# OpenStitching/stitching

Hardware: AMD Instinct MI355X
Metric: warped+blended Mpix/s (higher is better)
Workload: dtype u8/int16 (fixed-point remap, int32 pyramid sums, fp32 weights); 1 GPU; BASELINE config 2: 8 synthetic 4000x3000 frames, one ring; yaw step 38.9 deg = 0.58 hfov (42 % overlap; SURVEY 8(d) names 0.70 hfov); spherical warp + 5-band multiband blend, inputs resident in HBM; frames_per_gpu=8, panoramas_in_flight=2

## Files before the change

### include/stitching_amd_debug.h

```cpp
#ifndef STITCHING_AMD_DEBUG_H
#define STITCHING_AMD_DEBUG_H

#include "stitching_amd.h"

#ifdef __cplusplus
extern "C" {
#endif

int stx_debug_warp_maps(stx_ctx* ctx, int type, float scale, const float K[9], const float R[9], int w, int h, int which,
                        const int rect_xywh[4], stx_buf** out_xmap_f32, stx_buf** out_ymap_f32, int out_xywh[4]);

int stx_debug_feather_dist_cap(void);

#ifdef __cplusplus
}
#endif
#endif
```

### stitching_amd/_lib.py

```python
import ctypes as C
import os

from .stitching_error import StitchingError

_HERE = os.path.dirname(os.path.abspath(__file__))
LIB_PATH = os.environ.get("STITCHING_AMD_LIB") or os.path.join(_HERE, "libstitching_amd.so")

STX_OK = 0
WARP_PLANE, WARP_AFFINE, WARP_CYLINDRICAL, WARP_SPHERICAL = 0, 1, 2, 3
WARP_TYPE_IDS = {"plane": 0, "affine": 1, "cylindrical": 2, "spherical": 3, "fisheye": 4, "stereographic": 5,
                 "compressedPlaneA2B1": 6, "compressedPlaneA1.5B1": 7, "compressedPlanePortraitA2B1": 8,
                 "compressedPlanePortraitA1.5B1": 9, "paniniA2B1": 10, "paniniA1.5B1": 11, "paniniPortraitA2B1": 12,
                 "paniniPortraitA1.5B1": 13, "mercator": 14, "transverseMercator": 15}
INTER_NEAREST, INTER_LINEAR = 0, 1
BORDER_CONSTANT, BORDER_REFLECT = 0, 2
BLEND_NO, BLEND_FEATHER, BLEND_MULTIBAND = 0, 1, 2
U8, S16, F32 = 0, 1, 2
TRIG_MODES = {"exact": 0, "glibc": 1, "glibc-nofma": 2}
REMAP_MODES = {"q15": 0, "float": 1, "float-fma": 2}
PYRDOWN_MODES = {"scalar": 0, "simd-v": 1, "simd-hv": 3, "simd-v-fma": 5, "simd-hv-fma": 7}
GAIN_MAP_BOUNDED = 1
EXPOSURE_KINDS = {"gain": 1, "gain_blocks": 2, "channel": 3, "channel_blocks": 4}
EXPOSURE_SOLVERS = {"host": 0, "device": 1}
LU_NB, LU_MAX_N = 32, 16384
# ... 1 lines not shown
COLOR_SEAM_MAX_LENGTH, COLOR_SEAM_MAX_CROSS = 16384, 4096
FEATURES_MAX_SIDE, FEATURES_MAX_LEVELS, FEATURES_MAX_FEATURES = 32767, 16, 65536
MATCH_MAX_FEATURES, MATCH_MAX_ITERS = 65536, 4096
RAY_MAX_CAMERAS, RAY_MAX_MATCHES = 1024, 131072
CONTRIB_U8_BINARY = 1
STRIP_MASK_BITS = 2

EXPORTS = (
    "stx_version stx_last_error stx_set_trig_mode stx_get_trig_mode stx_set_remap_mode stx_get_remap_mode stx_set_pyrdown_mode stx_get_pyrdown_mode stx_device_count stx_ctx_create stx_ctx_destroy stx_ctx_sync "
    "stx_host_alloc stx_host_free stx_buf_from_host stx_buf_from_host_async stx_buf_alloc stx_buf_to_host stx_buf_to_host_async stx_buf_view stx_buf_info stx_buf_device_ptr stx_buf_free "
    "stx_warp_roi stx_warp_rois stx_warp stx_warp_image_and_mask stx_warp_batch stx_warp_batch_rects stx_warp_batch_gain stx_warp_batch_with_rois stx_warp_mask "
    "stx_gain_apply stx_block_gain_apply stx_block_gain_apply_batch stx_resize_linear_exact stx_resize_linear_exact_batch stx_seam_mask_resize stx_seam_mask_resize_batch stx_seam_mask_resize_batch_sub stx_timelapse_frame stx_result_roi stx_blend_create stx_blend_num_bands stx_blend_feed stx_blend_finish stx_blend_finish_ex "
    "stx_blend_destroy stx_blend_keep_weights stx_blend_use_weights stx_mb_weights_free stx_blend_set_band stx_blend_feed_ex stx_blend_contrib_rect stx_blend_export_contrib stx_blend_export_contribs "
    "stx_blend_build stx_blend_feed_contrib stx_blend_feed_contrib_ex stx_buf_flags stx_strip_rect stx_view_rect stx_strip_pack stx_strip_pack_batch stx_strip_pack_batch_ex stx_strip_bytes stx_strip_unpack stx_blend_feed_strips stx_comm_unique_id stx_comm_create stx_comm_exchange stx_comm_exchange_begin stx_comm_exchange_end stx_comm_exchange_begin_on stx_comm_exchange_end_on stx_comm_info stx_comm_destroy stx_prof_enable stx_prof_reset stx_prof_count stx_prof_get stx_mark stx_mark_elapsed_ms "
    "stx_exposure_feed stx_exposure_stats stx_exposure_solve stx_set_exposure_solver stx_get_exposure_solver stx_exposure_feed_ex stx_exposure_solve_device stx_lu_solve_device stx_seam_find stx_seam_schedule stx_color_seam_find stx_crop_lir stx_features_detect stx_match_features stx_ray_problem_create stx_ray_problem_eval stx_ray_problem_free "
    "stx_debug_warp_maps stx_debug_feather_dist_cap"
).split()

_lib = None


def build_hint():
    return "build it with `make -C stitching_amd/csrc` or `python -c 'import __graft_entry__ as g; g.build()'`"


def lib():
    global _lib
    if _lib is not None:
        return _lib
    if not os.path.exists(LIB_PATH):
        raise ImportError(f"{LIB_PATH} is missing: the HIP back end is not built ({build_hint()}). "
# ... 73 lines not shown
    L.stx_blend_feed_strips.argtypes = [vp, C.c_int, vpp, ip, ip, ip, ip, ip, C.c_int]
    L.stx_comm_unique_id.argtypes = [C.POINTER(C.c_ubyte)]
    L.stx_comm_create.argtypes = [vp, C.c_int, C.c_int, C.POINTER(C.c_ubyte), vpp]
    L.stx_comm_exchange.argtypes = [vp, C.c_int, ip, ip, C.POINTER(C.c_void_p), C.POINTER(C.c_size_t)]
    L.stx_comm_exchange_begin.argtypes = [vp, C.c_int, ip, ip, C.POINTER(C.c_void_p), C.POINTER(C.c_size_t)]
    L.stx_comm_exchange_end.argtypes = [vp]
    L.stx_comm_exchange_begin_on.argtypes = [vp, vp, C.c_int, ip, ip, C.POINTER(C.c_void_p), C.POINTER(C.c_size_t)]
    L.stx_comm_exchange_end_on.argtypes = [vp, vp]
    L.stx_comm_info.argtypes = [vp, ip]
    L.stx_comm_destroy.argtypes = [vp]
    L.stx_prof_enable.argtypes = [vp, C.c_int]
    L.stx_prof_reset.argtypes = [vp]
    L.stx_prof_count.argtypes = [vp, ip]
    L.stx_prof_get.argtypes = [vp, C.c_int, C.c_char_p, C.c_int, C.POINTER(C.c_int64), C.POINTER(C.c_double),
                               C.POINTER(C.c_double)]
    L.stx_debug_warp_maps.argtypes = [vp, C.c_int, C.c_float, fp, fp, C.c_int, C.c_int, C.c_int, ip, vpp, vpp, ip]
    llp, dp = C.POINTER(C.c_longlong), C.POINTER(C.c_double)
    L.stx_exposure_feed.argtypes = [vp, C.c_int, C.c_int, vpp, vpp, ip, C.c_int, C.c_int, dp, llp, dp]
    L.stx_exposure_stats.argtypes = [vp, C.c_int, C.c_int, vpp, vpp, ip, C.c_int, llp, ip, llp, dp]
    L.stx_exposure_solve.argtypes = [C.c_int, C.c_int, ip, dp, C.POINTER(C.c_ubyte), dp]
    L.stx_set_exposure_solver.argtypes = [C.c_int]
    L.stx_exposure_feed_ex.argtypes = [vp, C.c_int, C.c_int, vpp, vpp, ip, C.c_int, C.c_int, C.c_int, dp, llp, dp]
    L.stx_exposure_solve_device.argtypes = [vp, C.c_int, C.c_int, ip, dp, C.POINTER(C.c_ubyte), dp, dp]
    L.stx_lu_solve_device.argtypes = [vp, C.c_int, dp, dp, dp, dp]
    L.stx_seam_find.argtypes = [vp, C.c_int, C.c_int, ip, ip, vpp, vpp, dp]
    L.stx_seam_schedule.argtypes = [C.c_int, ip, ip, ip, ip, ip]
    L.stx_color_seam_find.argtypes = [vp, C.c_int, ip, ip, vpp, vpp, vpp, dp]
    L.stx_crop_lir.argtypes = [vp, vp, ip, ip, dp]
    L.stx_features_detect.argtypes = [vp, C.c_int, vpp, vpp, C.c_int, C.c_int, C.c_int, ip, ip, ip, ip, C.POINTER(C.c_byte), ip, ip, llp,
                                      C.POINTER(C.c_ubyte), dp]
# ... 19 lines not shown
```

### stitching_amd/csrc/stx_blend_fast.hip

```cpp
#include <algorithm>
#include <cstdlib>

#include "stx_blend_kernels.h"
#include "stx_device_math.h"

using namespace stxd;

namespace {

constexpr int L0_WAVES = 5;
constexpr float WEIGHT_EPS = 1e-5f;
constexpr float INV255 = 0.0039215688593685627f;
constexpr float INV256 = 0.00390625f;

#define STX_GAS __attribute__((address_space(1)))
template <class T> STX_DEV const STX_GAS T* gp(const T* p) { return (const STX_GAS T*)p; }
template <class T> STX_DEV STX_GAS T* gp(T* p) { return (STX_GAS T*)p; }

STX_DEV bool xcd_tile(const StxTileMap& M, uint32_t b, int& tx, int& ty)
{
    if (M.plain) {
        const uint32_t wy = M.tiles_x == 1 ? b : __umulhi(b, M.magic_tx);
        tx = (int)(b - wy * (uint32_t)M.tiles_x);
        ty = (int)wy;
// ... 929 lines not shown
        const uint32_t w0 = __builtin_amdgcn_alignbyte(d.y, d.x, sh), w1 = d.y >> (8u * sh);
        return ((w0 & (n >= 4 ? 0xffffffffu : (1u << (8 * n)) - 1u)) | (n > 4 ? w1 & 0xffu : 0u)) != 0u;
    }
    const uint32_t d0 = q[0], d1 = q[1], d2 = q[2];
    const uint32_t w0 = __builtin_amdgcn_alignbyte(d1, d0, sh), w1 = __builtin_amdgcn_alignbyte(d2, d1, sh), w2 = d2 >> (8u * sh);
    const uint32_t m0 = n >= 4 ? 0xffffffffu : (1u << (8 * n)) - 1u;
    const uint32_t m1 = n >= 8 ? 0xffffffffu : (n > 4 ? (1u << (8 * (n - 4))) - 1u : 0u);
    return ((w0 & m0) | (w1 & m1) | (n > 8 ? w2 & 0xffu : 0u)) != 0u;
}
template <bool L0>
STX_DEV bool occ_hit(const StxMbImage& im, int lv, int tile_x, int Y0)
{
    return occ_hit_f<L0>(im.occ[L0 ? 1 : lv], im.fx, im.fy, im.fw, im.fh, lv, tile_x, Y0);
}

template <bool WF>
STX_DEV void level0_epilogue_pk(const MbLevelK& P, int X0, int Y0, uint32_t (&acc)[2][3][4], uint32_t (&cnt)[2][4], const float (*ws)[8]);

template <bool L0, bool CONTRIB, bool EMIT, bool U8SRC>
STX_DEV void mb_level_fast_body(const MbLevelK& P)
{
    const int tid = threadIdx.x;
    const int lv = P.level;
    int tile_tx, tile_ty;
    if (!xcd_tile(P.tiles, blockIdx.x, tile_tx, tile_ty)) return;
    const int tile_x = P.x0 + tile_tx * 512, tile_y = P.y0 + tile_ty * LV_TH;
    const int X0 = tile_x + (tid & 63) * 8, Y0 = tile_y + __builtin_amdgcn_readfirstlane(tid >> 6) * 2;
    const bool active = X0 < P.x1 && Y0 < P.y1;

    int acc[2][8][3];
// ... 502 lines not shown
                for (int c = 0; c < 3; c++) w[j][c] = half_of(j) ? s16hi(v[r][c][pair_of(j)]) : s16lo(v[r][c][pair_of(j)]);
            uint32_t t[12];
#pragma unroll
            for (int j = 0; j < 8; j += 2) {
                t[(j >> 1) * 3 + 0] = pack16(w[j][0], w[j][1]);
                t[(j >> 1) * 3 + 1] = pack16(w[j][2], w[j + 1][0]);
                t[(j >> 1) * 3 + 2] = pack16(w[j + 1][1], w[j + 1][2]);
            }
            *reinterpret_cast<uint4*>(p16) = make_uint4(t[0], t[1], t[2], t[3]);
            *reinterpret_cast<uint4*>(p16 + 4) = make_uint4(t[4], t[5], t[6], t[7]);
            *reinterpret_cast<uint4*>(p16 + 8) = make_uint4(t[8], t[9], t[10], t[11]);
        }
    }
}

template <bool CONTRIB, bool DEFER = false>
__global__ __launch_bounds__(LV_THREADS) __attribute__((amdgpu_waves_per_eu(L0_WAVES, 8))) void mb_level0_pk_kernel(MbLevelK P)
{
    const int tid = threadIdx.x;
    int tile_tx, tile_ty;
    if (!xcd_tile(P.tiles, blockIdx.x, tile_tx, tile_ty)) return;
    const int tile_x = P.x0 + tile_tx * 512, tile_y = P.y0 + tile_ty * LV_TH;
    const int X0 = tile_x + (tid & 63) * 8, Y0 = tile_y + __builtin_amdgcn_readfirstlane(tid >> 6) * 2;
    const bool active = X0 < P.x1 && Y0 < P.y1;

    uint32_t acc[2][3][4];
    uint32_t cntb[2][2];
#pragma unroll
    for (int r = 0; r < 2; r++) {
#pragma unroll
        for (int k = 0; k < 4; k++) acc[r][0][k] = acc[r][1][k] = acc[r][2][k] = 0;
        cntb[r][0] = cntb[r][1] = 0;
    }
    uint32_t grey_seen = 0u;

    for (int base = 0; base < P.n_images; base += 64) {
        bool hit = false;
        {
            const int kk = base + (tid & 63);
            const StxMbImage& im = P.images[min(kk, P.n_images - 1)];
            const v4u f = *reinterpret_cast<const v4u_a4*>(&im.iw);
            const v4u ff = *reinterpret_cast<const v4u_a4*>(&im.fx);
            const uint8_t* const occp = im.occ[1];
            const int kind = CONTRIB ? im.kind : 0;
            int rx = (int)f.z, ry = (int)f.w, rw = (int)f.x, rh = (int)f.y;
            if (CONTRIB && kind == 1) { rx = (int)ff.x; ry = (int)ff.y; rw = (int)ff.z; rh = (int)ff.w; }
            hit = (kk < P.n_images) & (rx < tile_x + 512) & (rx + rw > tile_x) & (ry < Y0 + 2) & (ry + rh > Y0);
            if (hit) hit = occ_hit_f<true>(occp, (int)ff.x, (int)ff.y, (int)ff.z, (int)ff.w, 0, tile_x, Y0);
        }
        unsigned long long todo = __ballot(hit);
        while (todo) {
            const int k = base + (int)__builtin_ctzll(todo);
            todo &= todo - 1;
            const StxMbImage& im = P.images[k];
            if (!active) continue;
            if (CONTRIB && im.kind == 1) {
                const int cx0 = X0 - im.fx, cy0 = Y0 - im.fy;
                if ((unsigned)cx0 >= (unsigned)im.fw || (unsigned)cy0 >= (unsigned)im.fh) continue;
#pragma unroll
                for (int r = 0; r < 2; r++) {
#pragma unroll
                    for (int c = 0; c < 3; c++) {
                        const v4u gv = *reinterpret_cast<const STX_GAS v4u*>(
                            gp(im.g[0]) + c * im.g_plane[0] + ((uint32_t)(cy0 + r) * (uint32_t)im.g_stride[0] + (uint32_t)cx0));
                        acc[r][c][0] = unpk(pk(acc[r][c][0]) + pk(__builtin_amdgcn_perm(gv.y, gv.x, 0x05040100u)));
// ... 178 lines not shown
                            acc[r][j][c] += trunc_small(fmul((float)L, w));
                        }
                        ws[r][j] = fadd(ws[r][j], w);
                    }
            }
            if (live) level_epilogue<true>(P, X0, Y0, acc, ws);
        }
        g0 += nb;
    }
}

STX_DEV uint32_t min3u(uint32_t a, uint32_t b, uint32_t c) { return min(min(a, b), c); }
STX_DEV uint32_t max3u(uint32_t a, uint32_t b, uint32_t c) { return max(max(a, b), c); }

constexpr int LVPK_WAVES = 3;
__global__ __launch_bounds__(LV_THREADS) __attribute__((amdgpu_waves_per_eu(LVPK_WAVES, 8))) void mb_level_pk_kernel(MbLevelK P)
{
    const int tid = threadIdx.x;
    const int lv = P.level;
    int tile_tx, tile_ty;
    if (!xcd_tile(P.tiles, blockIdx.x, tile_tx, tile_ty)) return;
    const int tile_x = P.x0 + tile_tx * 512, tile_y = P.y0 + tile_ty * LV_TH;
    const int X0 = tile_x + (tid & 63) * 8, Y0 = tile_y + __builtin_amdgcn_readfirstlane(tid >> 6) * 2;
    const bool active = X0 < P.x1 && Y0 < P.y1;

    uint32_t acc[2][3][4];
    float ws[2][8];
#pragma unroll
    for (int r = 0; r < 2; r++) {
#pragma unroll
        for (int q = 0; q < 4; q++) acc[r][0][q] = acc[r][1][q] = acc[r][2][q] = 0;
#pragma unroll
        for (int j = 0; j < 8; j++) ws[r][j] = 0.f;
    }
    uint32_t ones = 0;
    uint32_t mixed = 0;

    for (int base = 0; base < P.n_images; base += 64) {
        bool hit = false;
        {
            const int kk = base + (tid & 63);
            const StxMbImage& im = P.images[min(kk, P.n_images - 1)];
            const v4u f = *reinterpret_cast<const v4u_a4*>(&im.fx);
            const uint8_t* const occp = im.occ[lv];
            const int rx = (int)f.x >> lv, ry = (int)f.y >> lv, rw = (int)f.z >> lv, rh = (int)f.w >> lv;
            hit = (kk < P.n_images) & (rx < tile_x + 512) & (rx + rw > tile_x) & (ry < Y0 + 2) & (ry + rh > Y0);
            if (hit) hit = occ_hit_f<false>(occp, (int)f.x, (int)f.y, (int)f.z, (int)f.w, lv, tile_x, Y0);
        }
        unsigned long long todo = __ballot(hit);
        while (todo) {
            const int k = base + (int)__builtin_ctzll(todo);
            todo &= todo - 1;
            const StxMbImage& im = P.images[k];
            if (!active) continue;
            int i_fx = im.fx, i_fy = im.fy, i_fw = im.fw, i_fh = im.fh, i_w1h = im.w1_f16;
            unsigned long long W_a = (unsigned long long)im.wt[lv], G0_a = (unsigned long long)im.g[lv], G1_a = (unsigned long long)im.g[lv + 1];
            uint32_t wst = (uint32_t)im.wt_stride[lv], g0s = (uint32_t)im.g_stride[lv], g1s = (uint32_t)im.g_stride[lv + 1];
            uint32_t g0p = (uint32_t)im.g_plane[lv], g1p = (uint32_t)im.g_plane[lv + 1];
            asm("" : "+s"(i_fx), "+s"(i_fy), "+s"(i_fw), "+s"(i_fh), "+s"(i_w1h), "+s"(W_a), "+s"(G0_a), "+s"(G1_a), "+s"(wst), "+s"(g0s),
                "+s"(g1s), "+s"(g0p), "+s"(g1p));
            const int lx0 = X0 - (i_fx >> lv), ly0 = Y0 - (i_fy >> lv);
            const int lw = i_fw >> lv, lh = i_fh >> lv;
            if ((unsigned)lx0 >= (unsigned)lw || (unsigned)ly0 >= (unsigned)lh) continue;
            const bool w_half = lv == 1 && i_w1h != 0;
// ... 164 lines not shown
#pragma unroll
    for (int r = 0; r < 2; r++) {
        if (Y0 + r >= P.y1) break;
#pragma unroll
        for (int c = 0; c < 3; c++) {
            v4u o;
            o.x = __builtin_amdgcn_perm(v[r][c][2], v[r][c][0], 0x05040100u);
            o.y = __builtin_amdgcn_perm(v[r][c][2], v[r][c][0], 0x07060302u);
            o.z = __builtin_amdgcn_perm(v[r][c][3], v[r][c][1], 0x05040100u);
            o.w = __builtin_amdgcn_perm(v[r][c][3], v[r][c][1], 0x07060302u);
            *reinterpret_cast<STX_GAS v4u*>(gp(P.out) + c * P.out_plane + (long long)(Y0 + r - P.out_y0) * P.out_stride + (X0 - P.out_x0)) = o;
        }
    }
}

bool launched_ok() { return hipGetLastError() == hipSuccess; }

}

bool stx_fast_mb_down_batch(stx_ctx* ctx, const StxMbImage* d_images, const StxMbImage* h_images, int n, int level, bool weights)
{
    int mw = 0, mh = 0;
    for (int i = 0; i < n; i++) {
        mw = std::max(mw, (h_images[i].fw >> level) >> 1);
        mh = std::max(mh, (h_images[i].fh >> level) >> 1);
    }
    if (n <= 0 || mw < 1 || mh < 1 || n > 65535) return false;
    StxTileMap M = stx_tile_map((mw + DN_TOW - 1) / DN_TOW, (mh + DN_TOH - 1) / DN_TOH, DN_BAND);
    constexpr int DN_PLAIN_FROM = 3;
    M.plain = level >= DN_PLAIN_FROM;
// ... 39 lines not shown
    return launched_ok();
}

static bool no_defer()
{
    static const bool off = getenv("STITCHING_AMD_NO_DEFER") != nullptr;
    return off;
}

bool stx_fast_mb_level(stx_ctx* ctx, const MbLevelK& K)
{
    MbLevelK KT;
    if (!fast_level_ok(K, &KT)) return false;
    dim3 grid(stx_tile_grid(KT.tiles), 1);
    hipStream_t st = ctx->stream;
    if (K.level == 0 && K.pk_ok && !K.emit && K.num_bands > 0) {
        static const unsigned pad_lds = getenv("STITCHING_AMD_L0_LDS") ? (unsigned)atoi(getenv("STITCHING_AMD_L0_LDS")) : 0u;
        if (K.has_contrib) hipLaunchKernelGGL(mb_level0_pk_kernel<true>, grid, dim3(LV_THREADS), pad_lds, st, KT);
        else hipLaunchKernelGGL(mb_level0_pk_kernel<false>, grid, dim3(LV_THREADS), pad_lds, st, KT);
    } else if (K.level == 0 && K.all_u8 && !K.has_contrib && !K.emit && K.num_bands > 0 && !no_defer()) {
        const int segs = std::min(KT.tiles.tiles_x, STX_DEFER_SEGS);
        const size_t seg_cap = (size_t)((KT.tiles.tiles_x + STX_DEFER_SEGS - 1) / STX_DEFER_SEGS) * (size_t)KT.tiles.tiles_y * (unsigned)LV_THREADS;
        const size_t counters = (size_t)STX_DEFER_SEGS * 128;
        KT.defer_segs = segs;
        StxDevBlock q;
        if (stx_dev_alloc(ctx, counters + seg_cap * (size_t)segs * sizeof(unsigned long long), &q) != STX_OK) return false;
        KT.defer_count = reinterpret_cast<unsigned*>(q.get());
        KT.defer_list = reinterpret_cast<unsigned long long*>(reinterpret_cast<uint8_t*>(q.get()) + counters);
        KT.defer_cap = (unsigned)seg_cap;
        hipMemsetAsync(q.get(), 0, counters, st);
        hipLaunchKernelGGL((mb_level0_pk_kernel<false, true>), grid, dim3(LV_THREADS), 0, st, KT);
        {
            StxProfScope prof2(ctx, "mb_level0_deferred", 0.0);
            hipLaunchKernelGGL(mb_level0_deferred_kernel, dim3(1024), dim3(256), 0, st, KT);
        }
        static const bool stats = getenv("STITCHING_AMD_DEFER_STATS") != nullptr;
        if (stats) {
            std::vector<unsigned> hc(counters / 4);
            hipStreamSynchronize(st);
            hipMemcpy(hc.data(), q.get(), counters, hipMemcpyDeviceToHost);
            unsigned long long tot = 0; unsigned mx = 0;
            for (int sgi = 0; sgi < segs; sgi++) { tot += hc[32 * sgi]; mx = std::max(mx, hc[32 * sgi]); }
            fprintf(stderr, "[stitching_amd] level-0 deferral: %llu of %llu patches queued (%d segments, fullest %u of %zu)\n", tot,
                    (unsigned long long)KT.tiles.tiles_x * KT.tiles.tiles_y * (unsigned long long)LV_THREADS, segs, mx, seg_cap);
        }
    } else if (K.emit) {
        if (K.level == 0) hipLaunchKernelGGL((mb_level_fast_kernel<true, false, true, false>), grid, dim3(LV_THREADS), 0, st, KT);
        else if (K.all_u8) hipLaunchKernelGGL((mb_level_fast_kernel<false, false, true, true>), grid, dim3(LV_THREADS), 0, st, KT);
        else hipLaunchKernelGGL((mb_level_fast_kernel<false, false, true, false>), grid, dim3(LV_THREADS), 0, st, KT);
    } else if (K.has_contrib) {
        if (K.level == 0) hipLaunchKernelGGL((mb_level_fast_kernel<true, true, false, false>), grid, dim3(LV_THREADS), 0, st, KT);
        else if (K.all_u8) hipLaunchKernelGGL((mb_level_fast_kernel<false, true, false, true>), grid, dim3(LV_THREADS), 0, st, KT);
        else hipLaunchKernelGGL((mb_level_fast_kernel<false, true, false, false>), grid, dim3(LV_THREADS), 0, st, KT);
    } else {
        static const bool no_pk_levels = getenv("STITCHING_AMD_NO_PK_LEVELS") != nullptr;
        if (K.level == 0 && K.all_u8 && K.num_bands > 0) hipLaunchKernelGGL((mb_level_fast_kernel<true, false, false, true>), grid, dim3(LV_THREADS), 0, st, KT);
        else if (K.level == 0) hipLaunchKernelGGL((mb_level_fast_kernel<true, false, false, false>), grid, dim3(LV_THREADS), 0, st, KT);
        else if (K.all_u8 && K.level < K.num_bands && !no_pk_levels) hipLaunchKernelGGL(mb_level_pk_kernel, grid, dim3(LV_THREADS), 0, st, KT);
        else if (K.all_u8) hipLaunchKernelGGL((mb_level_fast_kernel<false, false, false, true>), grid, dim3(LV_THREADS), 0, st, KT);
        else hipLaunchKernelGGL((mb_level_fast_kernel<false, false, false, false>), grid, dim3(LV_THREADS), 0, st, KT);
    }
    return launched_ok();
}
```

### stitching_amd/csrc/stx_blend_host.cpp

```cpp
#include <algorithm>
#include <climits>
#include <cmath>
#include <cstdlib>
#include <cstring>
#include <memory>

#include "stx_blend_kernels.h"
#include "stx_internal.h"

STX_EXPORT int stx_debug_feather_dist_cap(void) { return STX_FEATHER_DIST_CAP; }

STX_EXPORT int stx_result_roi(int n, const int* corners_xy, const int* sizes_wh, int out_xywh[4])
{
    if (n <= 0 || !corners_xy || !sizes_wh || !out_xywh) return stx_fail(STX_ERR_INVALID, "bad argument");
    int tlx = INT_MAX, tly = INT_MAX, brx = INT_MIN, bry = INT_MIN;
    for (int i = 0; i < n; i++) {
        tlx = std::min(tlx, corners_xy[2 * i]);
        tly = std::min(tly, corners_xy[2 * i + 1]);
        brx = std::max(brx, corners_xy[2 * i] + sizes_wh[2 * i]);
        bry = std::max(bry, corners_xy[2 * i + 1] + sizes_wh[2 * i + 1]);
    }
    out_xywh[0] = tlx; out_xywh[1] = tly; out_xywh[2] = brx - tlx; out_xywh[3] = bry - tly;
    return STX_OK;
}

constexpr size_t MB_FRONT_PAD = 64;

static void blender_release(stx_blender* b)
{
    for (stx_buf* h : b->held) stx_buf_release(h);
    b->held.clear();
    for (void* p : b->pyr_allocs) stx_dev_free(b->ctx, p);
    b->pyr_allocs.clear();
    for (void* p : b->wt_allocs) stx_dev_free(b->ctx, p);
    b->wt_allocs.clear();
    stx_mb_weights_release(b->keep);
    stx_mb_weights_release(b->adopted);
    b->keep = b->adopted = nullptr;
    b->d_all = nullptr;
    b->images.clear();
    b->built.clear();
    b->no_images.clear();
    b->feather_images.clear();
}

STX_EXPORT int stx_blend_create(stx_ctx* ctx, int kind, int num_bands, float sharpness, const int roi_xywh[4],
                                stx_blender** out)
{
    if (!roi_xywh || !out) return stx_fail(STX_ERR_INVALID, "null argument");
    if (!ctx && kind != STX_BLEND_MULTIBAND) return stx_fail(STX_ERR_INVALID, "ctx is null");
    if (ctx) STX_TRY(stx_set_device(ctx));
    if (kind < STX_BLEND_NO || kind > STX_BLEND_MULTIBAND) return stx_fail(STX_ERR_INVALID, "unknown blender kind %d", kind);
    int w = roi_xywh[2], h = roi_xywh[3];
    if (w <= 0 || h <= 0) return stx_fail(STX_ERR_INVALID, "empty destination roi %dx%d", w, h);
// ... 271 lines not shown
}

STX_EXPORT int stx_blend_feed(stx_blender* b, const stx_buf* img, const stx_buf* mask, int tlx, int tly)
{
    return stx_blend_feed_ex(b, img, mask, tlx, tly, -1);
}

static void mb_fill_common(const stx_blender* b, MbLevelK* K, const StxMbImage* d_images, int n, int lv)
{
    memset(K, 0, sizeof(*K));
    K->images = d_images; K->n_images = n; K->level = lv; K->num_bands = b->num_bands;
    K->pw = b->rw >> lv; K->ph = b->rh >> lv;
    K->all_u8 = 1;
}

static int mb_finish(stx_blender* b, stx_buf* pano, stx_buf* pmask, stx_buf* pano16)
{
    stx_ctx* ctx = b->ctx;
    const int nb = b->num_bands, n = (int)b->images.size();
    STX_TRY(mb_ensure_pyramids(b));
    StxMbImage* d_images = b->d_all;
    if (!d_images) STX_TRY(mb_upload(b, b->images.data(), n, &d_images));
    bool all_u8 = true, has_contrib = false, pk_ok = true;
    for (const StxMbImage& im : b->images) {
        if (im.kind == 0 && im.img0_is_s16) all_u8 = false;
        if (im.kind == 1) has_contrib = true;
        if ((im.kind == 0 && im.img0_is_s16) || !im.mask_binary) pk_ok = false;
    }
    int xb[STX_MAX_BANDS + 1], xe[STX_MAX_BANDS + 1];
    mb_level_regions(b, b->band_x0, b->band_x1, xb, xe);
    std::vector<short*> out(nb + 2, nullptr);
    std::vector<long long> ostride(nb + 2, 0), oplane(nb + 2, 0);
    static const bool no_fusion = getenv("STITCHING_AMD_NO_COARSE_FUSION") != nullptr;
    const bool fuse = nb >= 3 && !no_fusion;
    for (int lv = fuse ? nb - 2 : nb; lv >= 0; lv--) {
        MbLevelK K;
        mb_fill_common(b, &K, d_images, n, lv);
        K.all_u8 = all_u8 ? 1 : 0;
        K.has_contrib = has_contrib ? 1 : 0;
        K.pk_ok = pk_ok ? 1 : 0;
        K.x0 = xb[lv]; K.x1 = xe[lv]; K.y0 = 0; K.y1 = lv == 0 ? b->fh : b->rh >> lv;
        if (lv < nb) {
            K.up = out[lv + 1]; K.up_stride = ostride[lv + 1]; K.up_plane = oplane[lv + 1];
            K.up_x0 = xb[lv + 1]; K.up_y0 = 0;
        }
        if (lv == 0) {
            K.pano = pano->ptr; K.pano_stride = (long long)pano->stride;
            K.pmask = pmask->ptr; K.pmask_stride = (long long)pmask->stride;
            if (pano16) { K.pano16 = (short*)pano16->ptr; K.pano16_stride = (long long)pano16->stride; }
            K.pano_x0 = b->band_x0; K.pano_y0 = 0;
        } else {
            const int w = xe[lv] - xb[lv], ph = b->rh >> lv;
            const long long st = (long long)align_up((size_t)std::max(w, 1), 32);
            void* p = nullptr;
            STX_TRY(stx_dev_alloc(ctx, MB_FRONT_PAD + (size_t)st * ph * 3 * sizeof(short), &p));
            b->pyr_allocs.push_back(p);
// ... 46 lines not shown
        for (size_t h = 1; h < b->held.size(); h += 2)
            if (b->held[h]->ptr == im.mask0 && (long long)b->held[h]->stride == im.mask0_stride) k.mask = b->held[h];
        if (!k.mask) {
            for (StxMbKept& q : w->images) stx_buf_release(q.mask);
            w->images.clear();
            return;
        }
        stx_buf_retain(k.mask);
        k.mask0 = im.mask0; k.mask0_stride = im.mask0_stride; k.mask_binary = im.mask_binary; k.w1_f16 = im.w1_f16;
        k.iw = im.iw; k.ih = im.ih; k.ix = im.ix; k.iy = im.iy; k.fx = im.fx; k.fy = im.fy; k.fw = im.fw; k.fh = im.fh;
        k.left = im.left; k.top = im.top;
        for (int i = 1; i <= b->num_bands; i++) { k.wt[i] = im.wt[i]; k.wt_stride[i] = im.wt_stride[i]; k.occ[i] = im.occ[i]; }
        w->images.push_back(k);
    }
    w->allocs.swap(b->wt_allocs);
}

STX_EXPORT int stx_blend_keep_weights(stx_blender* b, stx_mb_weights** out)
{
    if (!b || !out) return stx_fail(STX_ERR_INVALID, "null argument");
    *out = nullptr;
    if (b->finished) return stx_fail(STX_ERR_STATE, "keep_weights after blend()");
    if (b->keep) return stx_fail(STX_ERR_STATE, "keep_weights was already called on this blender");
    if (b->images.empty() || !mb_weights_eligible(b, false)) return STX_OK;
    stx_mb_weights* w = new stx_mb_weights();
    w->ctx = b->ctx;
    w->refs = 2;
    b->keep = w;
    *out = w;
    return STX_OK;
// ... 16 lines not shown
            im.iw != k.iw || im.ih != k.ih || im.ix != k.ix || im.iy != k.iy || im.fx != k.fx || im.fy != k.fy || im.fw != k.fw ||
            im.fh != k.fh || im.left != k.left || im.top != k.top)
            return STX_OK;
        for (int l = 1; l <= b->num_bands; l++)
            if (im.wt_stride[l] != k.wt_stride[l]) return STX_OK;
    }
    STX_TRY(stx_set_device(b->ctx));
    for (size_t i = 0; i < b->images.size(); i++)
        for (int l = 1; l <= b->num_bands; l++) { b->images[i].wt[l] = w->images[i].wt[l]; b->images[i].occ[l] = w->images[i].occ[l]; }
    for (void* p : b->wt_allocs) stx_dev_free(b->ctx, p);
    b->wt_allocs.clear();
    b->d_all = nullptr;
    w->refs++;
    b->adopted = w;
    *out_adopted = 1;
    return STX_OK;
}

STX_EXPORT int stx_mb_weights_free(stx_mb_weights* w)
{
    stx_mb_weights_release(w);
    return STX_OK;
}

STX_EXPORT int stx_blend_set_band(stx_blender* b, int x0, int x1)
{
    if (!b) return stx_fail(STX_ERR_INVALID, "null argument");
    if (b->kind != STX_BLEND_MULTIBAND) return stx_fail(STX_ERR_UNSUPPORTED, "bands exist for the multi-band blender only");
    if (b->finished) return stx_fail(STX_ERR_STATE, "set_band after blend()");
    const int al = (1 << b->num_bands) - 1;
// ... 188 lines not shown
    NoGatherK K;
    K.imgs = (const NoImg*)d_tab; K.n = n; K.all_binary = all_binary ? 1 : 0;
    K.w = pano->w; K.h = pano->h;
    K.pano = pano->ptr; K.pano_stride = (long long)pano->stride; K.pmask = pmask->ptr; K.pmask_stride = (long long)pmask->stride;
    K.pano16 = p16 ? (short*)p16->ptr : nullptr; K.pano16_stride = p16 ? (long long)p16->stride : 0;
    return stx_launch_no_gather(ctx, K, bytes);
}

STX_EXPORT int stx_blend_finish_ex(stx_blender* b, stx_buf** out_pano_u8, stx_buf** out_mask_u8, stx_buf** out_pano_s16)
{
    if (!b) return stx_fail(STX_ERR_INVALID, "null argument");
    if (b->finished) return stx_fail(STX_ERR_STATE, "blend() was already called on this blender");
    if (!b->ctx) return stx_fail(STX_ERR_STATE, "geometry-only blender (created without a context)");
    STX_TRY(stx_set_device(b->ctx));
    stx_ctx* ctx = b->ctx;
    const int ow = b->kind == STX_BLEND_MULTIBAND ? b->band_x1 - b->band_x0 : b->rw, oh = b->kind == STX_BLEND_MULTIBAND ? b->fh : b->rh;
    StxBufRef p16, pmask, pano;
    const int rc = [&]() {
        STX_TRY(stx_buf_new(ctx, ow, oh, 3, STX_U8, &pano));
        STX_TRY(stx_buf_new(ctx, ow, oh, 1, STX_U8, &pmask));
        if (out_pano_s16) STX_TRY(stx_buf_new(ctx, ow, oh, 3, STX_S16, &p16));
        if (b->kind == STX_BLEND_MULTIBAND) return mb_finish(b, pano.get(), pmask.get(), p16.get());
        if (b->kind == STX_BLEND_NO) return no_finish(b, pano.get(), pmask.get(), p16.get());
        return feather_finish(b, pano.get(), pmask.get(), p16.get());
    }();
    if (rc == STX_OK) mb_hand_over_weights(b);
    b->finished = true;
    blender_release(b);
    STX_TRY(rc);
    if (out_pano_u8) *out_pano_u8 = pano.release();
// ... 21 lines not shown
```

### stitching_amd/csrc/stx_blend_kernels.h

```cpp
#pragma once
#include "stx_internal.h"

struct StxTileMap {
    int tiles_x, tiles_y, band_rows, band_tiles;
    unsigned magic_tx, magic_band;
    int plain;
};
inline StxTileMap stx_tile_map(int tiles_x, int tiles_y, int band_rows)
{
    StxTileMap m;
    m.tiles_x = tiles_x; m.tiles_y = tiles_y; m.band_rows = band_rows; m.band_tiles = band_rows * tiles_x;
    m.magic_tx = (unsigned)((1ull << 32) / (unsigned)tiles_x) + 1u;
    m.magic_band = (unsigned)((1ull << 32) / (unsigned)m.band_tiles) + 1u;
    m.plain = 0;
    return m;
}
inline unsigned stx_tile_grid(const StxTileMap& m)
{
    if (m.plain) return (unsigned)(m.tiles_x * m.tiles_y);
    const int bands = (m.tiles_y + m.band_rows - 1) / m.band_rows;
    return 8u * (unsigned)(((bands + 7) / 8) * m.band_tiles);
}

constexpr int STX_DEFER_SEGS = 256;
struct MbLevelK {
    const StxMbImage* images;
    int n_images, level, num_bands, pw, ph;
    int x0, x1, y0, y1;
    short* out; long long out_stride, out_plane; int out_x0, out_y0;
    const short* up; long long up_stride, up_plane; int up_x0, up_y0;
    int emit; float* out_w; long long out_w_stride;
    uint8_t* pano; long long pano_stride;
    uint8_t* pmask; long long pmask_stride;
    short* pano16; long long pano16_stride;
    int pano_x0, pano_y0;
    int has_contrib;
    int all_u8;
    StxTileMap tiles;
    int pk_ok;
    int defer_segs;
    unsigned long long* defer_list; unsigned* defer_count; unsigned defer_cap;
};

bool stx_fast_mb_down_batch(stx_ctx* ctx, const StxMbImage* d_images, const StxMbImage* h_images, int n, int level, bool weights);
bool stx_fast_mb_level(stx_ctx* ctx, const MbLevelK& K);

int stx_fast_mb_emit_class(const MbLevelK& K, MbLevelK* KT);
bool stx_fast_mb_emit_launch(stx_ctx* ctx, int cls, const MbLevelK* d_Ks, const MbLevelK* h_Ks, int count);
int stx_launch_mb_emit_batch(stx_ctx* ctx, const MbLevelK* d_Ks, const MbLevelK* h_Ks, const int* classes, int n, double bytes);
```

### stitching_amd/csrc/stx_internal.h

```cpp
#pragma once
#include <hip/hip_runtime.h>

#include <atomic>
#include <cstdarg>
#include <cstddef>
#include <cstdint>
#include <cstdio>
#include <map>
#include <memory>
#include <mutex>
#include <string>
#include <vector>

#include "../../include/stitching_amd.h"
#include "../../include/stitching_amd_debug.h"

#define STX_EXPORT extern "C" __attribute__((visibility("default")))
#define STX_MAX_BANDS 16

void stx_set_error(const char* fmt, ...);
int stx_fail(int code, const char* fmt, ...);

#define STX_HIP(call)                                                                                      \
    do {                                                                                                   \
// ... 33 lines not shown
    void* pinned = nullptr;
    size_t pinned_bytes = 0;
    uint32_t roi_seq = 0;
    uint8_t* stage = nullptr;
    size_t stage_bytes = 0, stage_off = 0;
    hipEvent_t stage_ev[4] = {};
    bool stage_ev_set[4] = {};
    int stage_seg = 0;
    bool prof_on = false;
    std::vector<StxProfEntry> prof;
    std::map<std::string, int> prof_index;
    std::vector<StxPendingEvent> prof_pending;
    std::vector<hipEvent_t> event_pool;
    hipEvent_t marks[16] = {};
    double* exp_sqrt = nullptr;
};

#define STX_STAGE_SEGS 4
int stx_dev_alloc(stx_ctx* ctx, size_t bytes, void** out);
int stx_stage_upload(stx_ctx* ctx, void* d, const void* h, size_t bytes);
void stx_dev_free(stx_ctx* ctx, void* p);
int stx_set_device(stx_ctx* ctx);
struct StxDevFree { stx_ctx* ctx; void operator()(void* p) const { stx_dev_free(ctx, p); } };
using StxDevBlock = std::unique_ptr<void, StxDevFree>;
inline int stx_dev_alloc(stx_ctx* ctx, size_t bytes, StxDevBlock* out)
{
    void* p = nullptr;
    STX_TRY(stx_dev_alloc(ctx, bytes, &p));
    *out = StxDevBlock(p, StxDevFree{ctx});
    return STX_OK;
// ... 218 lines not shown
struct stx_blender {
    stx_ctx* ctx = nullptr;
    int kind = 0, num_bands = 0;
    float sharpness = 0.02f;
    int rx = 0, ry = 0, rw = 0, rh = 0;
    int fw = 0, fh = 0;
    bool finished = false;
    std::vector<StxMbImage> images;
    std::vector<char> built;
    std::vector<stx_buf*> held;
    std::vector<void*> pyr_allocs;
    std::vector<void*> wt_allocs;
    stx_mb_weights* keep = nullptr;
    stx_mb_weights* adopted = nullptr;
    StxMbImage* d_all = nullptr;
    int band_x0 = 0, band_x1 = 0;
    int next_order = 0;
    int pyr_mode = 0;
    std::vector<NoImg> no_images;
    std::vector<FeatherImg> feather_images;
};
struct StxMbKept {
    stx_buf* mask;
    const uint8_t* mask0; long long mask0_stride; int mask_binary, w1_f16;
    int iw, ih, ix, iy, fx, fy, fw, fh, left, top;
    float* wt[STX_MAX_BANDS + 1]; long long wt_stride[STX_MAX_BANDS + 1];
    uint8_t* occ[STX_MAX_BANDS + 1];
};
struct stx_mb_weights {
    stx_ctx* ctx = nullptr;
    std::atomic<int> refs{1};
    int num_bands = 0, pyr_mode = 0;
    int rx = 0, ry = 0, rw = 0, rh = 0;
    std::vector<StxMbKept> images;
    std::vector<void*> allocs;
};
void stx_mb_weights_release(stx_mb_weights* w);
void mb_feed_rect(const stx_blender* b, int w, int h, int tlx, int tly, int* fx, int* fy, int* fw, int* fh);
bool mb_contrib_range(const stx_blender* b, int fx, int fw, int bx0, int bx1, int* sx0, int* sx1);
```

Baseline: 197,600 Mpix/s.

## Precompute per-tile image cover bitmasks when keeping weights and replay them in blend levels

When multiband weights are kept, a new cover kernel computes, for each level tile row, a 64-bit ballot mask of which images overlap it. Later blends that adopt those weights pass the table through MbLevelK, and the level-0 and level pk kernels read one scalar word instead of running per-image rect and occupancy tests. This cuts the per-tile image search in the blend kernels. In exchange it adds a small device table per level and a union field in MbLevelK, and the path applies only with adopted weights, at most 64 images and no contrib images.

```diff
diff --git a/include/stitching_amd_debug.h b/include/stitching_amd_debug.h
--- a/include/stitching_amd_debug.h
+++ b/include/stitching_amd_debug.h
@@ -12,6 +12,8 @@
 
 int stx_debug_feather_dist_cap(void);
 
+int stx_debug_blend_replayed(stx_ctx* ctx, int* out_launches);
+
 #ifdef __cplusplus
 }
 #endif
diff --git a/stitching_amd/_lib.py b/stitching_amd/_lib.py
--- a/stitching_amd/_lib.py
+++ b/stitching_amd/_lib.py
@@ -39,7 +39,7 @@
     "stx_blend_destroy stx_blend_keep_weights stx_blend_use_weights stx_mb_weights_free stx_blend_set_band stx_blend_feed_ex stx_blend_contrib_rect stx_blend_export_contrib stx_blend_export_contribs "
     "stx_blend_build stx_blend_feed_contrib stx_blend_feed_contrib_ex stx_buf_flags stx_strip_rect stx_view_rect stx_strip_pack stx_strip_pack_batch stx_strip_pack_batch_ex stx_strip_bytes stx_strip_unpack stx_blend_feed_strips stx_comm_unique_id stx_comm_create stx_comm_exchange stx_comm_exchange_begin stx_comm_exchange_end stx_comm_exchange_begin_on stx_comm_exchange_end_on stx_comm_info stx_comm_destroy stx_prof_enable stx_prof_reset stx_prof_count stx_prof_get stx_mark stx_mark_elapsed_ms "
     "stx_exposure_feed stx_exposure_stats stx_exposure_solve stx_set_exposure_solver stx_get_exposure_solver stx_exposure_feed_ex stx_exposure_solve_device stx_lu_solve_device stx_seam_find stx_seam_schedule stx_color_seam_find stx_crop_lir stx_features_detect stx_match_features stx_ray_problem_create stx_ray_problem_eval stx_ray_problem_free "
-    "stx_debug_warp_maps stx_debug_feather_dist_cap"
+    "stx_debug_warp_maps stx_debug_feather_dist_cap stx_debug_blend_replayed"
 ).split()
 
 _lib = None
@@ -143,6 +143,7 @@
     L.stx_prof_count.argtypes = [vp, ip]
     L.stx_prof_get.argtypes = [vp, C.c_int, C.c_char_p, C.c_int, C.POINTER(C.c_int64), C.POINTER(C.c_double),
                                C.POINTER(C.c_double)]
+    L.stx_debug_blend_replayed.argtypes = [vp, ip]
     L.stx_debug_warp_maps.argtypes = [vp, C.c_int, C.c_float, fp, fp, C.c_int, C.c_int, C.c_int, ip, vpp, vpp, ip]
     llp, dp = C.POINTER(C.c_longlong), C.POINTER(C.c_double)
     L.stx_exposure_feed.argtypes = [vp, C.c_int, C.c_int, vpp, vpp, ip, C.c_int, C.c_int, dp, llp, dp]
diff --git a/stitching_amd/csrc/stx_blend_fast.hip b/stitching_amd/csrc/stx_blend_fast.hip
--- a/stitching_amd/csrc/stx_blend_fast.hip
+++ b/stitching_amd/csrc/stx_blend_fast.hip
@@ -967,6 +967,37 @@
     return occ_hit_f<L0>(im.occ[L0 ? 1 : lv], im.fx, im.fy, im.fw, im.fh, lv, tile_x, Y0);
 }
 
+template <bool L0, bool CONTRIB>
+STX_DEV bool mb_tile_hit(const StxMbImage* images, int n_images, int lv, int tile_x, int Y0, int kk)
+{
+    const StxMbImage& im = images[min(kk, n_images - 1)];
+    bool hit;
+    if (L0) {
+        const v4u f = *reinterpret_cast<const v4u_a4*>(&im.iw);
+        const v4u ff = *reinterpret_cast<const v4u_a4*>(&im.fx);
+        const uint8_t* const occp = im.occ[1];
+        const int kind = CONTRIB ? im.kind : 0;
+        int rx = (int)f.z, ry = (int)f.w, rw = (int)f.x, rh = (int)f.y;
+        if (CONTRIB && kind == 1) { rx = (int)ff.x; ry = (int)ff.y; rw = (int)ff.z; rh = (int)ff.w; }
+        hit = (kk < n_images) & (rx < tile_x + 512) & (rx + rw > tile_x) & (ry < Y0 + 2) & (ry + rh > Y0);
+        if (hit) hit = occ_hit_f<true>(occp, (int)ff.x, (int)ff.y, (int)ff.z, (int)ff.w, 0, tile_x, Y0);
+    } else {
+        const v4u f = *reinterpret_cast<const v4u_a4*>(&im.fx);
+        const uint8_t* const occp = im.occ[lv];
+        const int rx = (int)f.x >> lv, ry = (int)f.y >> lv, rw = (int)f.z >> lv, rh = (int)f.w >> lv;
+        hit = (kk < n_images) & (rx < tile_x + 512) & (rx + rw > tile_x) & (ry < Y0 + 2) & (ry + rh > Y0);
+        if (hit) hit = occ_hit_f<false>(occp, (int)f.x, (int)f.y, (int)f.z, (int)f.w, lv, tile_x, Y0);
+    }
+    return hit;
+}
+
+typedef const unsigned long long __attribute__((address_space(4))) * StxCoverPtr;
+STX_DEV unsigned long long mb_cover_word(const MbLevelK& P, int tile_tx, int Y0)
+{
+    const int idx = __builtin_amdgcn_readfirstlane(((Y0 - P.y0) / LV_TH) * P.tiles.tiles_x + tile_tx);
+    return ((StxCoverPtr)P.cover)[idx];
+}
+
 template <bool WF>
 STX_DEV void level0_epilogue_pk(const MbLevelK& P, int X0, int Y0, uint32_t (&acc)[2][3][4], uint32_t (&cnt)[2][4], const float (*ws)[8]);
 
@@ -1499,7 +1530,7 @@
     }
 }
 
-template <bool CONTRIB, bool DEFER = false>
+template <bool CONTRIB, bool DEFER = false, bool REPLAY = false>
 __global__ __launch_bounds__(LV_THREADS) __attribute__((amdgpu_waves_per_eu(L0_WAVES, 8))) void mb_level0_pk_kernel(MbLevelK P)
 {
     const int tid = threadIdx.x;
@@ -1519,21 +1550,10 @@
     }
     uint32_t grey_seen = 0u;
 
-    for (int base = 0; base < P.n_images; base += 64) {
-        bool hit = false;
-        {
-            const int kk = base + (tid & 63);
-            const StxMbImage& im = P.images[min(kk, P.n_images - 1)];
-            const v4u f = *reinterpret_cast<const v4u_a4*>(&im.iw);
-            const v4u ff = *reinterpret_cast<const v4u_a4*>(&im.fx);
-            const uint8_t* const occp = im.occ[1];
-            const int kind = CONTRIB ? im.kind : 0;
-            int rx = (int)f.z, ry = (int)f.w, rw = (int)f.x, rh = (int)f.y;
-            if (CONTRIB && kind == 1) { rx = (int)ff.x; ry = (int)ff.y; rw = (int)ff.z; rh = (int)ff.w; }
-            hit = (kk < P.n_images) & (rx < tile_x + 512) & (rx + rw > tile_x) & (ry < Y0 + 2) & (ry + rh > Y0);
-            if (hit) hit = occ_hit_f<true>(occp, (int)ff.x, (int)ff.y, (int)ff.z, (int)ff.w, 0, tile_x, Y0);
-        }
-        unsigned long long todo = __ballot(hit);
+    for (int base = 0; base < (REPLAY ? 1 : P.n_images); base += 64) {
+        unsigned long long todo;
+        if (REPLAY) todo = mb_cover_word(P, tile_tx, Y0);
+        else todo = __ballot(mb_tile_hit<true, CONTRIB>(P.images, P.n_images, 0, tile_x, Y0, base + (tid & 63)));
         while (todo) {
             const int k = base + (int)__builtin_ctzll(todo);
             todo &= todo - 1;
@@ -1742,6 +1762,7 @@
 STX_DEV uint32_t max3u(uint32_t a, uint32_t b, uint32_t c) { return max(max(a, b), c); }
 
 constexpr int LVPK_WAVES = 3;
+template <bool REPLAY>
 __global__ __launch_bounds__(LV_THREADS) __attribute__((amdgpu_waves_per_eu(LVPK_WAVES, 8))) void mb_level_pk_kernel(MbLevelK P)
 {
     const int tid = threadIdx.x;
@@ -1764,18 +1785,10 @@
     uint32_t ones = 0;
     uint32_t mixed = 0;
 
-    for (int base = 0; base < P.n_images; base += 64) {
-        bool hit = false;
-        {
-            const int kk = base + (tid & 63);
-            const StxMbImage& im = P.images[min(kk, P.n_images - 1)];
-            const v4u f = *reinterpret_cast<const v4u_a4*>(&im.fx);
-            const uint8_t* const occp = im.occ[lv];
-            const int rx = (int)f.x >> lv, ry = (int)f.y >> lv, rw = (int)f.z >> lv, rh = (int)f.w >> lv;
-            hit = (kk < P.n_images) & (rx < tile_x + 512) & (rx + rw > tile_x) & (ry < Y0 + 2) & (ry + rh > Y0);
-            if (hit) hit = occ_hit_f<false>(occp, (int)f.x, (int)f.y, (int)f.z, (int)f.w, lv, tile_x, Y0);
-        }
-        unsigned long long todo = __ballot(hit);
+    for (int base = 0; base < (REPLAY ? 1 : P.n_images); base += 64) {
+        unsigned long long todo;
+        if (REPLAY) todo = mb_cover_word(P, tile_tx, Y0);
+        else todo = __ballot(mb_tile_hit<false, false>(P.images, P.n_images, lv, tile_x, Y0, base + (tid & 63)));
         while (todo) {
             const int k = base + (int)__builtin_ctzll(todo);
             todo &= todo - 1;
@@ -1970,6 +1983,21 @@
     }
 }
 
+static_assert(LV_WAVES == 1, "a cover word is the search of ONE wavefront: a tile of more wavefronts needs a word per wavefront");
+__global__ __launch_bounds__(LV_THREADS) void mb_cover_kernel(const StxMbImage* images, int n_images, int level, int x0, int y0, StxTileMap tiles,
+                                                              unsigned long long* cover)
+{
+    const int tid = threadIdx.x;
+    int tile_tx, tile_ty;
+    if (!xcd_tile(tiles, blockIdx.x, tile_tx, tile_ty)) return;
+    const int tile_x = x0 + tile_tx * 512, tile_y = y0 + tile_ty * LV_TH;
+    const int Y0 = tile_y + __builtin_amdgcn_readfirstlane(tid >> 6) * 2;
+    const bool hit = level == 0 ? mb_tile_hit<true, false>(images, n_images, 0, tile_x, Y0, tid & 63)
+                                : mb_tile_hit<false, false>(images, n_images, level, tile_x, Y0, tid & 63);
+    const unsigned long long word = __ballot(hit);
+    if ((tid & 63) == 0) cover[((Y0 - y0) / LV_TH) * tiles.tiles_x + tile_tx] = word;
+}
+
 bool launched_ok() { return hipGetLastError() == hipSuccess; }
 
 }
@@ -2039,10 +2067,14 @@
     if (!fast_level_ok(K, &KT)) return false;
     dim3 grid(stx_tile_grid(KT.tiles), 1);
     hipStream_t st = ctx->stream;
+    const bool replay = !K.emit && K.cover != nullptr && K.n_images <= 64 && !K.has_contrib;
+    bool replayed = false;
     if (K.level == 0 && K.pk_ok && !K.emit && K.num_bands > 0) {
         static const unsigned pad_lds = getenv("STITCHING_AMD_L0_LDS") ? (unsigned)atoi(getenv("STITCHING_AMD_L0_LDS")) : 0u;
         if (K.has_contrib) hipLaunchKernelGGL(mb_level0_pk_kernel<true>, grid, dim3(LV_THREADS), pad_lds, st, KT);
+        else if (replay) hipLaunchKernelGGL((mb_level0_pk_kernel<false, false, true>), grid, dim3(LV_THREADS), pad_lds, st, KT);
         else hipLaunchKernelGGL(mb_level0_pk_kernel<false>, grid, dim3(LV_THREADS), pad_lds, st, KT);
+        replayed = replay && !K.has_contrib;
     } else if (K.level == 0 && K.all_u8 && !K.has_contrib && !K.emit && K.num_bands > 0 && !no_defer()) {
         const int segs = std::min(KT.tiles.tiles_x, STX_DEFER_SEGS);
         const size_t seg_cap = (size_t)((KT.tiles.tiles_x + STX_DEFER_SEGS - 1) / STX_DEFER_SEGS) * (size_t)KT.tiles.tiles_y * (unsigned)LV_THREADS;
@@ -2054,7 +2086,9 @@
         KT.defer_list = reinterpret_cast<unsigned long long*>(reinterpret_cast<uint8_t*>(q.get()) + counters);
         KT.defer_cap = (unsigned)seg_cap;
         hipMemsetAsync(q.get(), 0, counters, st);
-        hipLaunchKernelGGL((mb_level0_pk_kernel<false, true>), grid, dim3(LV_THREADS), 0, st, KT);
+        if (replay) hipLaunchKernelGGL((mb_level0_pk_kernel<false, true, true>), grid, dim3(LV_THREADS), 0, st, KT);
+        else hipLaunchKernelGGL((mb_level0_pk_kernel<false, true>), grid, dim3(LV_THREADS), 0, st, KT);
+        replayed = replay;
         {
             StxProfScope prof2(ctx, "mb_level0_deferred", 0.0);
             hipLaunchKernelGGL(mb_level0_deferred_kernel, dim3(1024), dim3(256), 0, st, KT);
@@ -2081,9 +2115,29 @@
         static const bool no_pk_levels = getenv("STITCHING_AMD_NO_PK_LEVELS") != nullptr;
         if (K.level == 0 && K.all_u8 && K.num_bands > 0) hipLaunchKernelGGL((mb_level_fast_kernel<true, false, false, true>), grid, dim3(LV_THREADS), 0, st, KT);
         else if (K.level == 0) hipLaunchKernelGGL((mb_level_fast_kernel<true, false, false, false>), grid, dim3(LV_THREADS), 0, st, KT);
-        else if (K.all_u8 && K.level < K.num_bands && !no_pk_levels) hipLaunchKernelGGL(mb_level_pk_kernel, grid, dim3(LV_THREADS), 0, st, KT);
+        else if (K.all_u8 && K.level < K.num_bands && !no_pk_levels) {
+            if (replay) hipLaunchKernelGGL(mb_level_pk_kernel<true>, grid, dim3(LV_THREADS), 0, st, KT);
+            else hipLaunchKernelGGL(mb_level_pk_kernel<false>, grid, dim3(LV_THREADS), 0, st, KT);
+            replayed = replay;
+        }
         else if (K.all_u8) hipLaunchKernelGGL((mb_level_fast_kernel<false, false, false, true>), grid, dim3(LV_THREADS), 0, st, KT);
         else hipLaunchKernelGGL((mb_level_fast_kernel<false, false, false, false>), grid, dim3(LV_THREADS), 0, st, KT);
     }
+    if (replayed) ctx->blend_replayed++;
     return launched_ok();
 }
+
+void stx_fast_mb_cover_dims(int x0, int x1, int y0, int y1, int* tiles_x, int* tiles_y, int* band_rows)
+{
+    *tiles_x = (x1 - x0 + 511) / 512; *tiles_y = (y1 - y0 + LV_TH - 1) / LV_TH; *band_rows = LV_BAND;
+}
+
+bool stx_fast_mb_cover(stx_ctx* ctx, const StxMbImage* d_images, int n, int level, int x0, int x1, int y0, int y1, unsigned long long* cover)
+{
+    if (n < 1 || n > 64 || x1 <= x0 || y1 <= y0) return false;
+    int tx, ty, br;
+    stx_fast_mb_cover_dims(x0, x1, y0, y1, &tx, &ty, &br);
+    const StxTileMap M = stx_tile_map(tx, ty, br);
+    hipLaunchKernelGGL(mb_cover_kernel, dim3(stx_tile_grid(M), 1), dim3(LV_THREADS), 0, ctx->stream, d_images, n, level, x0, y0, M, cover);
+    return launched_ok();
+}
diff --git a/stitching_amd/csrc/stx_blend_host.cpp b/stitching_amd/csrc/stx_blend_host.cpp
--- a/stitching_amd/csrc/stx_blend_host.cpp
+++ b/stitching_amd/csrc/stx_blend_host.cpp
@@ -37,7 +37,7 @@
     stx_mb_weights_release(b->keep);
     stx_mb_weights_release(b->adopted);
     b->keep = b->adopted = nullptr;
-    b->d_all = nullptr;
+    b->d_all = b->d_gather = nullptr;
     b->images.clear();
     b->built.clear();
     b->no_images.clear();
@@ -339,6 +339,19 @@
     K->all_u8 = 1;
 }
 
+static int mb_level_y1(const stx_blender* b, int lv) { return lv == 0 ? b->fh : b->rh >> lv; }
+
+static const unsigned long long* mb_cover_for(const stx_mb_weights* w, const MbLevelK& K)
+{
+    if (!w || K.level < 0 || K.level > STX_MAX_BANDS || K.n_images > 64 || K.n_images != (int)w->images.size()) return nullptr;
+    const stx_mb_weights::Cover& c = w->cover[K.level];
+    int tx, ty, br;
+    stx_fast_mb_cover_dims(K.x0, K.x1, K.y0, K.y1, &tx, &ty, &br);
+    if (!c.table || c.x0 != K.x0 || c.x1 != K.x1 || c.y0 != K.y0 || c.y1 != K.y1 || c.tiles_x != tx || c.tiles_y != ty || c.band_rows != br)
+        return nullptr;
+    return c.table;
+}
+
 static int mb_finish(stx_blender* b, stx_buf* pano, stx_buf* pmask, stx_buf* pano16)
 {
     stx_ctx* ctx = b->ctx;
@@ -346,6 +359,7 @@
     STX_TRY(mb_ensure_pyramids(b));
     StxMbImage* d_images = b->d_all;
     if (!d_images) STX_TRY(mb_upload(b, b->images.data(), n, &d_images));
+    b->d_gather = d_images;
     bool all_u8 = true, has_contrib = false, pk_ok = true;
     for (const StxMbImage& im : b->images) {
         if (im.kind == 0 && im.img0_is_s16) all_u8 = false;
@@ -364,7 +378,8 @@
         K.all_u8 = all_u8 ? 1 : 0;
         K.has_contrib = has_contrib ? 1 : 0;
         K.pk_ok = pk_ok ? 1 : 0;
-        K.x0 = xb[lv]; K.x1 = xe[lv]; K.y0 = 0; K.y1 = lv == 0 ? b->fh : b->rh >> lv;
+        K.x0 = xb[lv]; K.x1 = xe[lv]; K.y0 = 0; K.y1 = mb_level_y1(b, lv);
+        if (b->adopted && !has_contrib) K.cover = mb_cover_for(b->adopted, K);
         if (lv < nb) {
             K.up = out[lv + 1]; K.up_stride = ostride[lv + 1]; K.up_plane = oplane[lv + 1];
             K.up_x0 = xb[lv + 1]; K.up_y0 = 0;
@@ -441,6 +456,21 @@
         w->images.push_back(k);
     }
     w->allocs.swap(b->wt_allocs);
+    if (b->images.size() > 64 || !b->d_gather) return;
+    int xb[STX_MAX_BANDS + 1], xe[STX_MAX_BANDS + 1];
+    mb_level_regions(b, b->band_x0, b->band_x1, xb, xe);
+    for (int lv = 0; lv <= b->num_bands - 3; lv++) {
+        stx_mb_weights::Cover c;
+        c.x0 = xb[lv]; c.x1 = xe[lv]; c.y0 = 0; c.y1 = mb_level_y1(b, lv);
+        if (c.x1 <= c.x0 || c.y1 <= c.y0) continue;
+        stx_fast_mb_cover_dims(c.x0, c.x1, c.y0, c.y1, &c.tiles_x, &c.tiles_y, &c.band_rows);
+        void* t = nullptr;
+        if (stx_dev_alloc(b->ctx, sizeof(unsigned long long) * (size_t)c.tiles_x * (size_t)c.tiles_y, &t) != STX_OK) return;
+        w->allocs.push_back(t);
+        c.table = (unsigned long long*)t;
+        if (!stx_fast_mb_cover(b->ctx, b->d_gather, (int)b->images.size(), lv, c.x0, c.x1, c.y0, c.y1, c.table)) return;
+        w->cover[lv] = c;
+    }
 }
 
 STX_EXPORT int stx_blend_keep_weights(stx_blender* b, stx_mb_weights** out)
@@ -487,6 +517,13 @@
     w->refs++;
     b->adopted = w;
     *out_adopted = 1;
+    return STX_OK;
+}
+
+STX_EXPORT int stx_debug_blend_replayed(stx_ctx* ctx, int* out_launches)
+{
+    if (!ctx || !out_launches) return stx_fail(STX_ERR_INVALID, "null argument");
+    *out_launches = ctx->blend_replayed;
     return STX_OK;
 }
 
@@ -705,6 +742,7 @@
     if (!b->ctx) return stx_fail(STX_ERR_STATE, "geometry-only blender (created without a context)");
     STX_TRY(stx_set_device(b->ctx));
     stx_ctx* ctx = b->ctx;
+    ctx->blend_replayed = 0;
     const int ow = b->kind == STX_BLEND_MULTIBAND ? b->band_x1 - b->band_x0 : b->rw, oh = b->kind == STX_BLEND_MULTIBAND ? b->fh : b->rh;
     StxBufRef p16, pmask, pano;
     const int rc = [&]() {
diff --git a/stitching_amd/csrc/stx_blend_kernels.h b/stitching_amd/csrc/stx_blend_kernels.h
--- a/stitching_amd/csrc/stx_blend_kernels.h
+++ b/stitching_amd/csrc/stx_blend_kernels.h
@@ -29,7 +29,7 @@
     int x0, x1, y0, y1;
     short* out; long long out_stride, out_plane; int out_x0, out_y0;
     const short* up; long long up_stride, up_plane; int up_x0, up_y0;
-    int emit; float* out_w; long long out_w_stride;
+    int emit; union { float* out_w; const unsigned long long* cover; }; long long out_w_stride;
     uint8_t* pano; long long pano_stride;
     uint8_t* pmask; long long pmask_stride;
     short* pano16; long long pano16_stride;
@@ -44,6 +44,8 @@
 
 bool stx_fast_mb_down_batch(stx_ctx* ctx, const StxMbImage* d_images, const StxMbImage* h_images, int n, int level, bool weights);
 bool stx_fast_mb_level(stx_ctx* ctx, const MbLevelK& K);
+void stx_fast_mb_cover_dims(int x0, int x1, int y0, int y1, int* tiles_x, int* tiles_y, int* band_rows);
+bool stx_fast_mb_cover(stx_ctx* ctx, const StxMbImage* d_images, int n, int level, int x0, int x1, int y0, int y1, unsigned long long* cover);
 
 int stx_fast_mb_emit_class(const MbLevelK& K, MbLevelK* KT);
 bool stx_fast_mb_emit_launch(stx_ctx* ctx, int cls, const MbLevelK* d_Ks, const MbLevelK* h_Ks, int count);
diff --git a/stitching_amd/csrc/stx_internal.h b/stitching_amd/csrc/stx_internal.h
--- a/stitching_amd/csrc/stx_internal.h
+++ b/stitching_amd/csrc/stx_internal.h
@@ -71,6 +71,7 @@
     std::vector<hipEvent_t> event_pool;
     hipEvent_t marks[16] = {};
     double* exp_sqrt = nullptr;
+    int blend_replayed = 0;
 };
 
 #define STX_STAGE_SEGS 4
@@ -319,6 +320,7 @@
     stx_mb_weights* keep = nullptr;
     stx_mb_weights* adopted = nullptr;
     StxMbImage* d_all = nullptr;
+    StxMbImage* d_gather = nullptr;
     int band_x0 = 0, band_x1 = 0;
     int next_order = 0;
     int pyr_mode = 0;
@@ -339,6 +341,8 @@
     int rx = 0, ry = 0, rw = 0, rh = 0;
     std::vector<StxMbKept> images;
     std::vector<void*> allocs;
+    struct Cover { int x0, x1, y0, y1, tiles_x, tiles_y, band_rows; unsigned long long* table; };
+    Cover cover[STX_MAX_BANDS + 1] = {};
 };
 void stx_mb_weights_release(stx_mb_weights* w);
 void mb_feed_rect(const stx_blender* b, int w, int h, int tlx, int tly, int* fx, int* fy, int* fw, int* fh);
```

After: 203,100 Mpix/s, median of 6. +2.8%, better.
